# gooofy/zerovox

Hardware: AMD Instinct MI355X
Metric: audio samples/sec + RTF, 128-phoneme zero-shot synth @22.05kHz, 1/2/4/8 GPU (higher is better)
Workload: dtype f16+bf16

## Files before the change

### zerovox_amd/build.py

```python
import os
import subprocess
import sys

HERE = os.path.dirname(os.path.abspath(__file__))
CSRC = os.path.join(HERE, "csrc")
LIB = os.path.join(HERE, "libzvx.so")
KTEST_SRC = os.path.join(os.path.dirname(HERE), "tests", "native", "zvx_ktest.hip")
KTEST_LIB = os.path.join(HERE, "libzvx_ktest.so")
SOURCES = ["gemm.hip", "resstream.hip", "pairstream.hip", "narrowstage.hip", "attention.hip", "ops.hip", "spectral.hip", "zvx.hip"]
UNITS = [("gemm", "gemm.hip", ["-DZVX_GEMM_PART=1"]), ("gemm_resfuse", "gemm.hip", ["-DZVX_GEMM_PART=2"])] + \
        [(s_[:-4], s_, []) for s_ in SOURCES[1:]]
FLAGS = ["--offload-arch=gfx950", "-O3", "-std=c++17", "-fPIC", "-Wall", "-Wno-unused-function", "-Wno-inline-asm"]
EXTRA_FLAGS = {"gemm.hip": ["-fno-honor-nans"], "pairstream.hip": ["-fno-honor-nans"], "narrowstage.hip": ["-fno-honor-nans"], "resstream.hip": ["-fno-honor-nans"] + (["-DRS_PROFILE"] if os.environ.get("ZVX_RS_PROFILE_BUILD") else [])}


def _stale(target, deps):
    if not os.path.exists(target):
        return True
    t = os.path.getmtime(target)
    return any(os.path.getmtime(d) > t for d in deps)


def _parse_resources(text):
    import re
    res, cur = {}, None
    keys = {"TotalSGPRs": "sgprs", "VGPRs": "vgprs", "AGPRs": "agprs", "ScratchSize [bytes/lane]": "scratch", "Occupancy [waves/SIMD]": "occupancy",
            "SGPRs Spill": "sgpr_spill", "VGPRs Spill": "vgpr_spill", "LDS Size [bytes/block]": "lds"}
    for line in text.splitlines():
        m = re.search(r"remark:\s+Function Name: (\S+)", line)
        if m:
            cur = res.setdefault(m.group(1), {})
            continue
        m = re.search(r"remark:\s+([A-Za-z \[\]/]+): (\d+)", line)
        if m and cur is not None and m.group(1).strip() in keys:
            cur[keys[m.group(1).strip()]] = int(m.group(2))
    return res


def resources():
    import json
    out = {}
    for stem, _src, _defs in UNITS:
        f = os.path.join(CSRC, stem + ".resources.json")
        if os.path.exists(f):
            out.update(json.load(open(f)))
    return out


def build(force: bool = False, verbose: bool = True) -> str:
    hipcc = os.environ.get("HIPCC", "/opt/rocm/bin/hipcc")
    headers = [os.path.join(CSRC, "zvx_kernels.h"), os.path.join(CSRC, "mfma_util.h"), os.path.join(CSRC, "stream_plan.h"), os.path.join(os.path.dirname(HERE), "include", "zvx.h")]
    def compile_one(unit):
        stem, src, defs = unit
        s = os.path.join(CSRC, src)
        o = os.path.join(CSRC, stem + ".o")
        rj = os.path.join(CSRC, stem + ".resources.json")
        if force or _stale(o, [s] + headers) or not os.path.exists(rj):
            cmd = [hipcc] + FLAGS + EXTRA_FLAGS.get(src, []) + defs + ["-Rpass-analysis=kernel-resource-usage", "-c", s, "-o", o]
            if verbose:
                print(" ".join(cmd), flush=True)
            p = subprocess.run(cmd, stderr=subprocess.PIPE, text=True)
            lines, keep, skip = p.stderr.splitlines(), [], 0
            for l in lines:
                if "[-Rpass-analysis=kernel-resource-usage]" in l:
                    skip = 2
                elif skip and (l.lstrip().startswith("|") or (l.strip()[:1].isdigit() and " | " in l)):
# ... 43 lines not shown
```

### zerovox_amd/csrc/gemm.hip

```cpp
#include "mfma_util.h"
#include "zvx_kernels.h"

#include <cstring>
#include <type_traits>

#ifndef ZVX_GEMM_PART
#define ZVX_GEMM_PART 0
#endif
#define ZVX_PART_MAIN (ZVX_GEMM_PART != 2)
#define ZVX_PART_RESFUSE (ZVX_GEMM_PART != 1)
#if ZVX_GEMM_PART == 2
extern thread_local bool zvx_gemm_dry_run;
#else
thread_local hipEvent_t zvx_gemm_ev_start = nullptr, zvx_gemm_ev_stop = nullptr;
thread_local bool zvx_gemm_dry_run = false;
#endif
#define g_dry_run zvx_gemm_dry_run

#define ZVX_LAUNCH(...) do { if (!g_dry_run) ZVX_DISPATCH(__VA_ARGS__); } while (0)

namespace zvx {


#define PITCH 80
// ... 1650 lines not shown
        if (a.ntaps == 3) { ZVX_RFP_MODE(3) }
        if (a.ntaps == 7) { ZVX_RFP_MODE(7) }
        if constexpr (C <= 32) { if (a.ntaps == 11) { ZVX_RFP_MODE(11) } }
    }
#undef ZVX_RFP_MODE
#undef ZVX_RFP
    return false;
}

int launch_resfuse(GemmArgs a, hipStream_t stream) {
    if (a.dtype == DT_F32 || !a.Wp || !a.Wp2 || a.N != a.K || a.nheads != 1 || a.wout > 0) return -1;
    if (!(a.ntaps == 3 || a.ntaps == 7 || a.ntaps == 11)) return -1;
    int h1 = 0;
    for (int i = 0; i < a.ntaps; i++) { const int d = a.dv1[i] < 0 ? -a.dv1[i] : a.dv1[i]; if (d > h1) h1 = d; }
    if (h1 > 32) return -1;
    a.halo_l = a.halo_r = h1;
    a.fused = 1;
    if (a.N == 128 && a.no_pairstream != 1) {
        const int h2 = (a.ntaps - 1) / 2, dil = a.dv1[1] - a.dv1[0];
        bool ok = a.alpha == 1.f && a.bias_mode == 1 && !a.post_scale && (!a.out || a.out_dtype == a.dtype) && a.res_mode == 2 && a.res_dtype == a.dtype &&
                  a.res == a.X && a.r_bs == a.x_bs && a.ldr == a.ldx && (!a.accum || a.accum_dtype == a.dtype) && (a.act == ACT_NONE || a.act == ACT_LRELU) &&
                  (a.accum_mode || a.out_scale == 1.f) && a.in_len == a.out_len;
        for (int t = 0; t < a.ntaps; t++) ok = ok && a.dv[t] == t - h2 && a.dv1[t] == (t - h2) * dil;
        if (ok) {
            PairArgs p;
            memset(&p, 0, sizeof p);
            p.X = a.X; p.x_bs = a.x_bs; p.ldx = a.ldx; p.W1 = a.Wp2; p.W2 = a.Wp; p.b1 = a.bias1; p.b2 = a.bias;
            p.C = a.N; p.ntaps = a.ntaps; p.dil = dil;
            p.out = a.out; p.o_bs = a.o_bs; p.ldo = a.ldo;
            p.accum = a.accum; p.a_bs = a.a_bs; p.lda = a.lda; p.accum_mode = a.accum ? a.accum_mode : 0;
            p.slope1 = a.slope1; p.res_inv_slope = a.res_inv_slope; p.out_scale = a.out_scale; p.slope = a.act == ACT_LRELU ? a.slope : 1.f;
            p.f16 = a.dtype == DT_F16;
            p.len = a.out_len; p.M = a.M; p.nbatch = a.nbatch; p.force = a.no_pairstream == 2;
            if (launch_pairstream(p, stream, g_dry_run)) return 23;
        }
    }
    {
        if (a.N == 32 && launch_resfuse_persist_c<32>(a, stream)) return 16;
        if (a.N == 64 && a.ntaps != 11 && launch_resfuse_persist_c<64>(a, stream)) return 17;
        if (a.N == 64 && a.ntaps == 11 && launch_resfuse_persist_c<64, 1>(a, stream)) return 17;
    }
    return -1;
}
#endif
#if ZVX_PART_MAIN

struct Variant { const char* name; int dt, bm, bn; };
static const Variant kVariants[] = {
    {"gemm_bf16_128x128", DT_BF16, 128, 128}, {"gemm_bf16_256x64", DT_BF16, 256, 64},
    {"gemm_bf16_256x32", DT_BF16, 256, 32},   {"gemm_f32_128x128", DT_F32, 128, 128},
    {"gemm_f32_256x64", DT_F32, 256, 64},     {"gemm_f32_256x32", DT_F32, 256, 32},
    {"convslab_bf16_128x256", DT_BF16, 128, 256}, {"convslab_bf16_256x128", DT_BF16, 256, 128},
    {"convslab_bf16_256x64", DT_BF16, 256, 64},   {"convslab_bf16_256x32", DT_BF16, 256, 32},
    {"(unused)", DT_BF16, 0, 0}, {"resfuse_bf16_c8", DT_BF16, 256, 8}, {"resfuse_bf16_c16", DT_BF16, 256, 16}, {"resfuse_bf16_c128", DT_BF16, 64, 128},
    {"convreg_bf16_c32", DT_BF16, 512, 32},       {"convreg_bf16_c64", DT_BF16, 256, 64},
    {"resfuse_bf16_c32", DT_BF16, 256, 32},       {"resfuse_bf16_c64", DT_BF16, 128, 64},
    {"gemm_bf16_64x64", DT_BF16, 64, 64},         {"gemm_f32_64x64", DT_F32, 64, 64},
    {"resstream_bf16_c32", DT_BF16, 64, 32},      {"resstream_bf16_c64", DT_BF16, 32, 64},
    {"convslab_bf16_128x128", DT_BF16, 128, 128},
    {"pairstream_bf16_c128", DT_BF16, 128, 128},
    {"narrowstage_c16", DT_BF16, 256, 16}, {"narrowstage_c8", DT_BF16, 512, 8},
    {"conv2d_persist_c32", DT_BF16, 384, 32}, {"conv2d_persist_c64", DT_BF16, 256, 64},
    {"conv2d_s2_c32", DT_BF16, 256, 64}, {"conv2d_s2_c64", DT_BF16, 128, 128},
    {"rb2fuse_bf16_c32", DT_BF16, 256, 32}, {"rb2fuse_bf16_c64", DT_BF16, 256, 64},
};
const char* gemm_variant_name(int id) { return kVariants[id].name; }
int gemm_num_variants() { return (int)(sizeof(kVariants) / sizeof(kVariants[0])); }


template <int BM, int BN, int WM, int WN, int MINW, int R, int EPI = -1>
static void launch_slab_variant(const GemmArgs& a, dim3 grid, size_t lds, hipStream_t stream) {
    const bool fullk = a.K % SLAB_KC == 0 && a.K2 == 0;
    if constexpr (R == 0 || EPI == -1 || EPI == ZVX_EPI(0, 0, 1) || EPI == ZVX_EPI_FLIP) {
        if (a.dtype == DT_F16) {
            if (fullk) ZVX_LAUNCH((convslab_kernel<BM, BN, WM, WN, true, MINW, R, EPI, 64, true>), grid, dim3(256), lds, stream, a);
            else if constexpr (EPI != ZVX_EPI_FLIP) ZVX_LAUNCH((convslab_kernel<BM, BN, WM, WN, false, MINW, R, EPI, 64, true>), grid, dim3(256), lds, stream, a);
            return;
        }
    }
    if constexpr (EPI < 0 || !(EPI & 16)) {
        if (fullk) ZVX_LAUNCH((convslab_kernel<BM, BN, WM, WN, true, MINW, R, EPI>), grid, dim3(256), lds, stream, a);
        else if constexpr (EPI != ZVX_EPI_FLIP) ZVX_LAUNCH((convslab_kernel<BM, BN, WM, WN, false, MINW, R, EPI>), grid, dim3(256), lds, stream, a);
    }
}

int gemm_epi_mode_of(const GemmArgs& a) {
    if (a.alpha == 1.f && !a.post_scale && a.out && a.out_dtype != a.dtype && a.dtype != DT_F32 && a.out_dtype != DT_F32 && !a.out_split3 && a.bias_mode == 1 && a.bias &&
        (a.act == ACT_NONE || a.act == ACT_LRELU) && !a.res_mode && !(a.accum && a.accum_mode) && a.out_scale == 1.f && a.K % SLAB_KC == 0 && !a.K2) return ZVX_EPI_FLIP;
    if (a.alpha != 1.f || a.post_scale || (a.out && a.out_dtype != a.dtype) || a.dtype == DT_F32 || a.out_split3 || a.bias_mode == 2) return -1;
    const int am = a.accum ? a.accum_mode : 0;
    if (a.dtype == DT_F16 && a.out && !am && a.act == ACT_NONE && a.res_mode <= 1 && (!a.res_mode || a.res_dtype == DT_F16) && (a.res_mode || a.out_scale != 1.f) &&
        (a.bias_mode == 0 || a.bias)) return ZVX_EPI_DEC(a.res_mode ? 1 : 0);
    if (a.bias_mode != 1 || !a.bias) return -1;
    if (a.act != ACT_NONE && a.act != ACT_LRELU) return -1;
    if (a.res_mode && (a.res_mode != 2 || a.res_dtype != a.dtype)) return -1;
    if (am && a.accum_dtype != a.dtype) return -1;
    if (!am && a.out_scale != 1.f) return -1;
    if (!a.out && !(am & 2)) return -1;
    const int e = ZVX_EPI(a.res_mode ? 1 : 0, am, a.out ? 1 : 0);
    switch (e) {
        case ZVX_EPI(0, 0, 1): case ZVX_EPI(1, 0, 1): case ZVX_EPI(1, 2, 0): case ZVX_EPI(1, 3, 0): case ZVX_EPI(1, 1, 1): return e;
    }
    return -1;
}

static int launch_convslab(GemmArgs a, hipStream_t stream) {
    const bool bflat_hint = a.bflat != 0;
// ... 247 lines not shown
```

### zerovox_amd/csrc/zvx.hip

```cpp
#include "../../include/zvx.h"
#include "zvx_kernels.h"
#include "stream_plan.h"

#include <dlfcn.h>
#include <math.h>
#include <cmath>
#include <rccl/rccl.h>
#include <stdarg.h>
#include <stdio.h>
#include <string.h>

#include <algorithm>
#include <map>
#include <sstream>
#include <stdexcept>
#include <string>
#include <vector>

using namespace zvx;

namespace {

struct ZvxError : std::runtime_error {
    int code;
// ... 28 lines not shown
struct zvx_ctx {
    int device = 0;
    hipStream_t stream = nullptr;
    hipStream_t main0 = nullptr;
    hipStream_t comm_stream = nullptr;
    hipStream_t voc_aux[2] = {nullptr, nullptr};
    hipEvent_t voc_ev[3] = {nullptr, nullptr, nullptr};
    int voc_overlap_maxb = 1 << 20;
    int voc_overlap_frames = 28672;
    hipStream_t front_stream = nullptr;
    hipEvent_t ev_front_done = nullptr, ev_mel_free = nullptr, ev_main_join = nullptr;
    int front_overlap = 1;
    bool mel_free_pending = false;
    bool front_dirty_main = true;
    struct HostSlot { void* p = nullptr; size_t cap = 0; hipEvent_t ready = nullptr, done = nullptr; bool pending = false; int B = 0, pcm16 = 0; long stride = 0, need = 0; };
    HostSlot host_slot[2];
    int host_next = 0, host_last = -1;
    hipStream_t copy_stream = nullptr;
    bool copy_is_comm = false;
    hipStream_t aux_stream = nullptr;
    hipEvent_t ev_aux[2] = {nullptr, nullptr};
    int va_overlap_maxb = 1 << 20;
    ncclComm_t comm = nullptr;
    int rank = 0, world = 1;
    hipEvent_t ev_compute = nullptr;
    std::map<const void*, hipEvent_t> gather_fence;
    std::string err;
    std::map<std::string, std::string> cfg;
    std::map<std::string, Tensor> tensors;
    std::vector<float> host_blob;
    std::map<std::string, DevBuf> bufs;
    std::map<const void*, const void*> packed;
    std::map<const void*, const void*> pair_packed;
    int dt = DT_BF16;
    int H = 0, emb_dim = 0, punct_dim = 0, n_phone_rows = 0, n_punct_rows = 0, max_txt_len = 0, max_mel_len = 0;
    int enc_layers = 0, enc_heads = 0, ffn_dim = 0, ffn_k0 = 0, ffn_k1 = 0, vp_dim = 0, vp_k = 0, n_bins = 0;
    int dec_layers = 0, dec_heads = 0, dec_scln = 0, n_mels = 0, hop = 0, res_dim = 0, dec_kind = 0, rn_asp = 1;
    std::vector<int> rn_layers, rn_filters, voc_rates, voc_ksizes, voc_rb_k;
    std::vector<std::vector<int>> voc_rb_d;
    int voc_resblock = 1, voc_c0 = 0;
    int B = 0, Tmax = 0, Lmax = 0;
    std::vector<int> T_host, mel_len_host;
    std::vector<int> in_stage;
    bool have_features = false, have_mel = false;
    int profile = 0;
    int profile_only = -1;
    int rs_prof = 0;
    int enc_split = 0;
    const void* fft_xs_ready = nullptr;
    int norm_fuse_maxb = 1 << 20;
    int dec_sc_fuse = 1;
    int dec_flat = 1;
    int voc_f16_stages = -1;
    int voc_h16_ok = -1;
    int voc_f16 = 1;
    int dec_f16 = 1;
    int use_attn_f32 = 1;
    int use_flash = 1;
    int use_resstream = 1;
    int rs_seg_min = 0;
    int spk_s2_fuse = 1;
    int spk_pool_fuse = 1;
    int slab_small = 2, slab_flat = 1;
    int poison_pads = 0;
    int sat_check = 0;
    unsigned long long* sat_count_dev() { return (unsigned long long*)buf("sat.count", 64); }
    void sat_scan(const void* x, int dt, long bs, int ld, int B, int rows_max, const int* rows, int C) {
        if (sat_check && x && dt == DT_F16) launch_count_sat16(x, bs, ld, B, rows_max, rows, C, sat_count_dev(), stream);
    }
    int use_rb2fuse = 1;
    int use_stagefuse = 1;
    struct NsWeights { void* W = nullptr; float* bias = nullptr; int woff[18] = {0}; };
    std::map<std::string, NsWeights> ns_weights;
    int use_pairstream = 1;
    int shape_log = 0;
    int max_frames = 1 << 18;
    int out_rate = 0;
    struct RsBank { int L = 0, M = 0, half = 0, T = 0, pitch = 0; const float* dev = nullptr; };
    std::map<std::pair<int, int>, RsBank> rs_banks;
    std::map<int, const double*> lim_wins;
    std::map<int, LoudCoef> loud_coefs;
    struct DnTables { int n_fft = 0, log2n = 0, win_length = 0; const float* twid = nullptr; const float* win = nullptr; const double* win2 = nullptr; double den_min = 0; };
    DnTables dn_tab;
    void* join_host = nullptr;
    size_t join_host_cap = 0;
    void* join_pinned(size_t bytes) {
        if (bytes > join_host_cap) {
            if (join_host) { HIPCHK(hipStreamSynchronize(stream)); HIPCHK(hipHostFree(join_host)); join_host = nullptr; join_host_cap = 0; }
            const size_t cap = bytes + bytes / 8 + 256;
            HIPCHK(hipHostMalloc(&join_host, cap, hipHostMallocDefault));
            join_host_cap = cap;
        }
        return join_host;
    }
    hipEvent_t stage_ev[ZVX_T_COUNT][2];
    bool stage_used[ZVX_T_COUNT];
    float stage_ms[ZVX_T_COUNT];
    std::vector<GemmEvent> pending;
    std::vector<zvx_kernel_stat> stats;
    std::string tag = "other";
    std::map<std::string, zvx_kernel_stat> tagstats;
    std::map<std::string, zvx_kernel_stat> namedstats;
    std::vector<hipEvent_t> event_pool;
    std::vector<zvx_stream*> streams;

    int cfg_int(const char* k) const {
// ... 1081 lines not shown
struct VocStage {
    int i, Cin, Cout, rows_in, rows;
    const int* len_in; const int* len;
    int dt_in, dt;
    float next_slope;
};

struct RbConv { std::string name; const Tensor* w = nullptr; const void* packed = nullptr; const float* bias = nullptr; };
struct RbWeights { std::string name; std::vector<RbConv> c1, c2; };
RbWeights voc_rb_weights(zvx_ctx* c, const VocCall& v, const VocStage& s, int j) {
    RbWeights w;
    w.name = "voc.rb" + std::to_string(s.i * v.nk + j);
    auto conv = [&](const char* which, int t) {
        RbConv r;
        r.name = w.name + which + std::to_string(t);
        r.w = &voc_weight(c, r.name + "_w", s.dt);
        auto it = c->packed.find(r.w->dev);
        if (it != c->packed.end()) r.packed = it->second;
        r.bias = c->pf(r.name + "_b");
        return r;
    };
    for (int t = 0; t < (int)c->voc_rb_d[j].size(); t++) {
        if (c->voc_resblock == 1) { w.c1.push_back(conv(".c1_", t)); w.c2.push_back(conv(".c2_", t)); }
        else w.c1.push_back(conv(".c_", t));
    }
    return w;
}

struct StageClose { int accum_mode; bool writes_out; };
StageClose stage_close(int j, int nk) {
    if (nk == 1) return {0, true};
    return {j == 0 ? 2 : (j < nk - 1 ? 3 : 1), j == nk - 1};
}
template <typename Args>
void close_stage(Args& a, const StageClose& cl, const VocCall& v, const VocStage& s) {
    a.accum = cl.accum_mode ? v.XS : nullptr; a.accum_mode = cl.accum_mode; a.a_bs = (long)s.rows * s.Cout; a.lda = s.Cout;
    if (cl.writes_out) { a.out = v.A; a.out_scale = 1.0f / v.nk; a.slope = s.next_slope; }
    else a.out = nullptr;
    if constexpr (std::is_same<Args, GemmArgs>::value) { a.accum_dtype = s.dt; if (cl.writes_out) a.act = ACT_LRELU; }
}

void voc_conv_pre(zvx_ctx* c, const VocCall& v, const void* vin, int dt) {
    const int nm = c->n_mels, Pmax = v.Pmax;
    const int* P_d = v.lens_d + v.B;
    GemmArgs a = gemm_base(dt);
    a.X = vin; a.x_bs = (long)Pmax * nm; a.ldx = nm; a.W = voc_weight(c, "voc.pre_w", dt).dev; a.ldw = nm; a.w_ts = (long)c->voc_c0 * nm;
    a.M = Pmax; a.N = c->voc_c0; a.K = nm; a.nbatch = v.B; a.in_len = P_d; a.out_len = P_d;
    set_taps_1d(a, c->t("voc.pre_w").dim(0), 1);
    a.bias = c->pf("voc.pre_b"); a.bias_mode = 1; a.act = ACT_LRELU; a.slope = 0.1f;
    a.out = v.A; a.o_bs = (long)Pmax * c->voc_c0; a.ldo = c->voc_c0;
    c->gemm(a);
}

void voc_upsample(zvx_ctx* c, const VocCall& v, const VocStage& s) {
    const int u = c->voc_rates[s.i], ku = c->voc_ksizes[s.i], B = v.B, Cin = s.Cin, Cout = s.Cout, rows_in = s.rows_in, dt_in = s.dt_in;
    const std::string up = "voc.up" + std::to_string(s.i);
    GemmArgs a = gemm_base(dt_in);
    a.out_dtype = s.dt;
    a.X = v.A; a.x_bs = (long)rows_in * Cin; a.ldx = Cin; a.ldw = Cin;
    a.M = rows_in; a.K = Cin; a.nbatch = B; a.in_len = s.len_in; a.out_len = s.len_in;
    a.bias_mode = 1; a.act = ACT_LRELU; a.slope = 0.1f;
    a.o_bs = (long)rows_in * u * Cout; a.ldo = u * Cout;
    if (dt_in != DT_F32 && c->has(up + "_wlo")) {
        const int hc = (u / 2) * Cout;
        a.N = hc; a.ntaps = 2; a.w_ts = (long)hc * Cin; a.flops = 2.0 * B * (double)rows_in * Cin * Cout * ku / 2;
        a.W = voc_weight(c, up + "_wlo", dt_in).dev; a.dv[0] = -1; a.dv[1] = 0;
        a.bias = c->pf(up + "_b"); a.out = v.X0;
        c->gemm(a);
        a.Wp = nullptr;
        a.W = voc_weight(c, up + "_whi", dt_in).dev; a.dv[0] = 0; a.dv[1] = 1;
        a.bias = c->pf(up + "_b") + hc; a.out = (char*)v.X0 + (size_t)hc * c->es();
        c->gemm(a);
    } else {
        a.W = voc_weight(c, up + "_w", dt_in).dev; a.w_ts = (long)u * Cout * Cin; a.N = u * Cout;
        a.ntaps = 3; a.dv[0] = -1; a.dv[1] = 0; a.dv[2] = 1;
        a.bias = c->pf(up + "_b"); a.out = v.X0;
        a.flops = 2.0 * B * (double)rows_in * Cin * Cout * ku;
        c->gemm(a);
    }
}

const zvx_ctx::NsWeights& voc_narrow_weights(zvx_ctx* c, const VocCall& v, const VocStage& s) {
    const int Cout = s.Cout, nk = v.nk;
    const std::string key = "voc.ns." + std::to_string(s.i) + (s.dt == DT_F16 ? ".h16" : "");
    auto it = c->ns_weights.find(key);
    if (it != c->ns_weights.end()) return it->second;
    zvx_ctx::NsWeights nw;
    int nfrag = 0;
    for (int j = 0; j < nk; j++) for (int q = 0; q < 6; q++) { nw.woff[6 * j + q] = nfrag; nfrag += narrowstage_steps(Cout, c->voc_rb_k[j]); }
    nw.W = c->buf(key + ".w", (size_t)nfrag * 1024);
    nw.bias = c->fbuf(key + ".b", (size_t)6 * nk * Cout);
    for (int j = 0; j < nk; j++) {
        const RbWeights w = voc_rb_weights(c, v, s, j);
        for (int t = 0; t < 3; t++)
            for (int q = 0; q < 2; q++) {
                const RbConv& cv = q ? w.c2[t] : w.c1[t];
                if (cv.w->dims.size() != 3 || cv.w->dim(0) != c->voc_rb_k[j] || cv.w->dim(1) != Cout || cv.w->dim(2) != Cout) fail(ZVX_E_MANIFEST, "weights: '%s' has an unexpected shape", cv.name.c_str());
                const int ci = 6 * j + 2 * t + q;
                launch_pack_narrow(cv.w->dev, c->voc_rb_k[j], Cout, (char*)nw.W + (size_t)nw.woff[ci] * 1024, c->stream);
                HIPCHK(hipMemcpyAsync(nw.bias + (size_t)ci * Cout, cv.bias, (size_t)Cout * 4, hipMemcpyDeviceToDevice, c->stream));
            }
    }
    return c->ns_weights.emplace(key, nw).first->second;
}

bool voc_narrow_stage(zvx_ctx* c, const VocCall& v, const VocStage& s) {
    const int Cout = s.Cout, nk = v.nk, rows = s.rows;
    if (!c->use_stagefuse || c->sat_check || c->voc_resblock != 1 || s.dt == DT_F32 || (Cout != 16 && Cout != 8) || nk < 1 || nk > 3) return false;
    for (int j = 0; j < nk; j++) if (c->voc_rb_d[j].size() != 3) return false;
// ... 1807 lines not shown
void zvx_destroy(zvx_ctx* c) {
    if (!c) return;
    (void)hipSetDevice(c->device);
    if (c->front_stream) (void)hipStreamSynchronize(c->front_stream);
    if (c->stream) (void)hipStreamSynchronize(c->stream);
    while (!c->streams.empty()) stream_free(c->streams.back());
    zvx_comm_destroy(c);
    for (int i = 0; i < 2; i++) { if (c->arena[i].p) (void)hipHostFree(c->arena[i].p); if (c->arena[i].ev) (void)hipEventDestroy(c->arena[i].ev); }
    if (c->copy_stream && !c->copy_is_comm) { (void)hipStreamSynchronize(c->copy_stream); (void)hipStreamDestroy(c->copy_stream); }
    for (auto& hs : c->host_slot) { if (hs.p) (void)hipHostFree(hs.p); if (hs.ready) (void)hipEventDestroy(hs.ready); if (hs.done) (void)hipEventDestroy(hs.done); }
    if (c->join_host) (void)hipHostFree(c->join_host);
    for (int i = 0; i < 2; i++) if (c->voc_aux[i]) { (void)hipStreamSynchronize(c->voc_aux[i]); (void)hipStreamDestroy(c->voc_aux[i]); }
    for (int i = 0; i < 3; i++) if (c->voc_ev[i]) (void)hipEventDestroy(c->voc_ev[i]);
    if (c->aux_stream) { (void)hipStreamSynchronize(c->aux_stream); (void)hipStreamDestroy(c->aux_stream); (void)hipEventDestroy(c->ev_aux[0]); (void)hipEventDestroy(c->ev_aux[1]); }
    if (c->front_stream) {
        (void)hipStreamSynchronize(c->front_stream); (void)hipStreamDestroy(c->front_stream);
        (void)hipEventDestroy(c->ev_front_done); (void)hipEventDestroy(c->ev_mel_free); (void)hipEventDestroy(c->ev_main_join);
    }
    for (auto& kv : c->bufs) if (kv.second.base) (void)hipFree(kv.second.base);
    for (auto e : c->event_pool) (void)hipEventDestroy(e);
    if (c->stream) {
        for (int s = 0; s < ZVX_T_COUNT; s++) { (void)hipEventDestroy(c->stage_ev[s][0]); (void)hipEventDestroy(c->stage_ev[s][1]); }
        (void)hipStreamDestroy(c->stream);
    }
    delete c;
}

const char* zvx_last_error(const zvx_ctx* c) { return c ? c->err.c_str() : g_create_error.c_str(); }

namespace {

struct Switch { const char* key; int zvx_ctx::*v; bool (*ok)(int64_t); };
bool flag(int64_t v) { return v == 0 || v == 1; }
bool count(int64_t v) { return v >= 0 && v <= INT32_MAX; }
const Switch kSwitches[] = {
    {"profile", &zvx_ctx::profile, [](int64_t v) { return v >= 0 && v <= 2; }},
    {"profile_only", &zvx_ctx::profile_only, [](int64_t v) { return v >= -1 && v < gemm_num_variants(); }},
    {"shape_log", &zvx_ctx::shape_log, flag},
    {"rs_prof", &zvx_ctx::rs_prof, flag},
    {"f16_sat_check", &zvx_ctx::sat_check, flag},
    {"poison_pads", &zvx_ctx::poison_pads, flag},
    {"max_frames", &zvx_ctx::max_frames, [](int64_t v) { return v >= 1 && v <= (1 << 24); }},
    {"enc_split", &zvx_ctx::enc_split, [](int64_t v) { return v >= 0 && v <= 2; }},
    {"attn_f32", &zvx_ctx::use_attn_f32, flag},
    {"flash", &zvx_ctx::use_flash, flag},
    {"front_overlap", &zvx_ctx::front_overlap, [](int64_t v) { return v >= 0 && v <= 2; }},
    {"va_overlap_maxb", &zvx_ctx::va_overlap_maxb, count},
    {"dec_f16", &zvx_ctx::dec_f16, flag},
    {"dec_flat", &zvx_ctx::dec_flat, flag},
    {"dec_sc_fuse", &zvx_ctx::dec_sc_fuse, flag},
    {"norm_fuse_maxb", &zvx_ctx::norm_fuse_maxb, count},
    {"voc_f16", &zvx_ctx::voc_f16, flag},
    {"voc_f16_stages", &zvx_ctx::voc_f16_stages, [](int64_t v) { return v >= -1 && v <= INT32_MAX; }},
    {"voc_overlap_maxb", &zvx_ctx::voc_overlap_maxb, count},
    {"voc_overlap_frames", &zvx_ctx::voc_overlap_frames, count},
    {"stagefuse", &zvx_ctx::use_stagefuse, flag},
    {"rb2fuse", &zvx_ctx::use_rb2fuse, flag},
    {"resstream", &zvx_ctx::use_resstream, flag},
    {"rs_seg_min", &zvx_ctx::rs_seg_min, [](int64_t v) { return v >= -1 && v <= INT32_MAX; }},
    {"pairstream", &zvx_ctx::use_pairstream, [](int64_t v) { return v == -1 || v == 0 || v == 1 || v == 3; }},
    {"slab_small", &zvx_ctx::slab_small, [](int64_t v) { return (v & ~32) >= 0 && (v & ~32) <= 2; }},
    {"slab_flat", &zvx_ctx::slab_flat, flag},
    {"spk_pool_fuse", &zvx_ctx::spk_pool_fuse, flag},
    {"spk_s2_fuse", &zvx_ctx::spk_s2_fuse, flag},
    {"out_rate", &zvx_ctx::out_rate, count},
};
const Switch* find_switch(const char* key) {
    for (const Switch& s : kSwitches) if (!strcmp(s.key, key)) return &s;
    return nullptr;
}

}

int64_t zvx_get_int(const zvx_ctx* c, const char* key) {
    if (!c || !key) return -1;
    if (const Switch* s = find_switch(key)) return c->*s->v;
    const std::string k(key);
    if (k == "precision") return c->dt == DT_F32 ? 1 : 0;
    if (k == "hidden") return c->H;
    if (k == "n_mels") return c->n_mels;
    if (k == "hop") return c->hop;
    if (k == "device") return c->device;
    if (k == "dec_kind") return c->dec_kind;
    if (k == "Lmax") return c->Lmax;
    if (k == "f16_sat_events") {
        zvx_ctx* m = const_cast<zvx_ctx*>(c);
        unsigned long long n = 0;
        if (hipSetDevice(m->device) != hipSuccess) return -1;
        try { unsigned long long* d = m->sat_count_dev(); m->sync(); if (hipMemcpy(&n, d, sizeof n, hipMemcpyDeviceToHost) != hipSuccess) return -1; } catch (...) { return -1; }
        return (int64_t)n;
    }
    if (k == "host_slot") return c->host_last;
    if (k.rfind("variant_id:", 0) == 0) { for (int i = 0; i < gemm_num_variants(); i++) if (k.substr(11) == gemm_variant_name(i)) return i; return -1; }
    auto it = c->cfg.find(k);
    if (it != c->cfg.end()) return atoll(it->second.c_str());
    return -1;
}

zvx_status zvx_set_int(zvx_ctx* c, const char* key, int64_t value) {
    return guarded(c, [&] {
        if (!key) fail(ZVX_E_INVALID, "key is NULL");
        const Switch* s = find_switch(key);
        if (!s) fail(ZVX_E_INVALID, "unknown option '%s'", key);
        if (!s->ok(value)) fail(ZVX_E_INVALID, "option '%s' does not take the value %lld", key, (long long)value);
        const std::string k(key);
        if (k == "out_rate" && value) {
// ... 550 lines not shown
```

### zerovox_amd/csrc/zvx_kernels.h

```cpp
#pragma once
#include <hip/hip_runtime.h>
#include <hip/hip_ext.h>
#include <stdint.h>
#include <atomic>
#include <mutex>
#include <set>
#include <utility>

extern thread_local hipEvent_t zvx_gemm_ev_start, zvx_gemm_ev_stop;
#define ZVX_DISPATCH(kernel, grid, block, lds, stream, ...) \
    do { if (zvx_gemm_ev_start) hipExtLaunchKernelGGL(kernel, grid, block, lds, stream, zvx_gemm_ev_start, zvx_gemm_ev_stop, 0, __VA_ARGS__); \
         else hipLaunchKernelGGL(kernel, grid, block, lds, stream, __VA_ARGS__); } while (0)

namespace zvx {

inline void profile_events(hipEvent_t start, hipEvent_t stop) { zvx_gemm_ev_start = start; zvx_gemm_ev_stop = stop; }

typedef unsigned short bf16_t;

enum DType { DT_F32 = 0, DT_BF16 = 1, DT_F16 = 2 };
static inline size_t dtype_size(int dt) { return dt == DT_F32 ? 4 : 2; }
inline int num_cus() {
    static const int n = [] { int dev = 0, v = 0; if (hipGetDevice(&dev) != hipSuccess || hipDeviceGetAttribute(&v, hipDeviceAttributeMultiprocessorCount, dev) != hipSuccess || v <= 0) v = 256; return v; }();
    return n;
// ... 64 lines not shown
const char* gemm_variant_name(int id);
int gemm_num_variants();

struct StreamArgs {
    const void* X; long x_bs; int ldx;
    const void* W1[3]; const void* W2[3];
    const float* b1[3]; const float* b2[3];
    int dil[3];
    int C, ntaps, npair;
    void* out; long o_bs; int ldo;
    void* accum; long a_bs; int lda; int accum_mode;
    float slope1, res_inv_slope, out_scale, slope;
    const int* len; int M, nbatch;
    int S, nseg;
    int dX0, dT, dX[3];
    double flops;
    long long* prof;
    int seg_min;
    int f16;
};
int launch_resstream(StreamArgs a, hipStream_t stream, bool dry_run);

struct PairArgs {
    const void* X; long x_bs; int ldx;
    const void* W1; const void* W2;
    const float* b1; const float* b2;
    int C, ntaps, dil;
    void* out; long o_bs; int ldo;
    void* accum; long a_bs; int lda; int accum_mode;
    float slope1, res_inv_slope, out_scale, slope;
    const int* len; int M, nbatch;
    int force;
    int f16;
    int S, nseg, DX, DT, G0;
    long long* prof;
};
bool launch_pairstream(PairArgs a, hipStream_t stream, bool dry_run);

struct StageArgs {
    const void* X; long x_bs; int ldx;
    const void* W;
    int woff[18];
    const float* bias;
    int C, nk, ks[3], dil[3][3];
    void* out; long o_bs; int ldo;
    float slope1, res_inv_slope, slope;
    const int* len; int M, nbatch;
    int f16;
};
bool launch_narrowstage(const StageArgs& a, hipStream_t stream, bool dry_run);
int narrowstage_steps(int C, int k);
void launch_pack_narrow(const void* w16 , int k, int C, void* out, hipStream_t s);

struct FlashArgs {
    const void* qk; long qk_bs; int ldq; int k_off;
    const void* vt; long vt_bs; int ldv;
    void* out; long o_bs; int ldo;
    const int* len; int L, D, nheads, nbatch;
    float scale;
    int f16;
    long long* prof;
};
bool launch_flash_attention(const FlashArgs& a, hipStream_t stream, bool dry_run);
struct AttnF32Args {
    const float* qkv; long bs; int ld; int q_off, k_off, v_off;
    float* out; long o_bs; int ldo;
    unsigned short* planes; int planes_C;
    int planes_f16;
    const int* len; int L, D, nheads, nbatch;
    float scale;
};
bool launch_attention_f32(const AttnF32Args& a, hipStream_t stream, bool dry_run);

void launch_instnorm_fused(const void* x, int x_dt, int ldx, void* y, int y_dt, int ldy, int B, int Lmax, const int* L, int C, float eps,
                           float* mean, float* rstd, const float* gamma, const float* beta, long g_bs, int one_plus, int act, float slope, hipStream_t s);
void launch_transpose16(const void* in, int ld_in, void* out, int ld_out, int B, int rows, int C, hipStream_t s, const int* len = nullptr);
void launch_f32_to_bf16(const float* in, bf16_t* out, size_t n, hipStream_t s);
void launch_zero_tail_cols(void* x, int es, long ld, long bs, int B, int rows, int cols, const int* len, hipStream_t s);
void launch_cast(const void* in, int in_dt, void* out, int out_dt, size_t n, hipStream_t s);

void launch_split3(const float* x, int ldx, void* out, int B, int rows_max, const int* rows, int C, hipStream_t s, int f16 = 0);
void launch_split3_weights(const float* w, void* out, long nrows, int K, hipStream_t s, int f16 = 0, float scale = 1.f);
void launch_absmax(const float* x, size_t n, float* out , hipStream_t s);

void launch_embed(const int* phoneme, const int* puncts, const float* emb, int emb_dim, const float* pemb,
                  int pemb_dim, const float* pe, float* out, int B, int Tmax, const int* T, hipStream_t s);

void launch_layernorm(const void* x, int x_dt, int ldx, void* y, int y_dt, int ldy, int B, int rows_max,
                      const int* rows, int C, int mode, float eps, const float* gamma, const float* beta,
                      const float* bg, long bg_bs, const float* post_add, hipStream_t s, void* split_planes = nullptr, int planes_f16 = 0);

void launch_softmax_rows(const float* scores, int lds, void* P, int p_dt, int ldp, int nbatch, int nheads,
                         int Lmax, const int* len, hipStream_t s);

void launch_rowdot(const float* x, int ldx, const float* w, float bias, float* out, int B, int Tmax,
                   const int* T, int C, hipStream_t s);

void launch_bucket_embed_add(const float* pred, const float* table, int nbins, float* x, int ldx, int C,
                             int* idx_out, int B, int Tmax, const int* T, hipStream_t s);

void launch_durations(const int* forced, const float* logd, int* dur, int* cum, int* mel_len, int B, int Tmax,
                      const int* T, hipStream_t s);

void launch_bucket_embed_add_ctl(const float* pred, const float* shift, const float* range, const float* target, const float* table,
                                 int nbins, float* x, int ldx, int C, int* idx_out, int B, int Tmax, const int* T, hipStream_t s);
void launch_durations_q16(const int* forced, const float* logd, const int* q, int* dur, int* cum, int* mel_len, int B, int Tmax,
// ... 159 lines not shown
```

Before: 348.2 million.

## Add dedicated transposed-conv upsample kernel for small vocoder stages

Adds a new MFMA kernel for the vocoder's transposed-convolution upsample (kernel = 2×rate). It stages input rows in LDS and streams prepacked weights through a register ring, then fuses bias, leaky ReLU and output packing with a permlane swap for coalesced stores. It is enabled by default for stages with Cin ≤ 256 and replaces the generic GEMM path there. It relies on a packed weight layout found via c->packed, and falls back to the GEMM path if the shape is unsupported.

```diff
diff --git a/zerovox_amd/build.py b/zerovox_amd/build.py
--- a/zerovox_amd/build.py
+++ b/zerovox_amd/build.py
@@ -7,11 +7,11 @@
 LIB = os.path.join(HERE, "libzvx.so")
 KTEST_SRC = os.path.join(os.path.dirname(HERE), "tests", "native", "zvx_ktest.hip")
 KTEST_LIB = os.path.join(HERE, "libzvx_ktest.so")
-SOURCES = ["gemm.hip", "resstream.hip", "pairstream.hip", "narrowstage.hip", "attention.hip", "ops.hip", "spectral.hip", "zvx.hip"]
+SOURCES = ["gemm.hip", "resstream.hip", "pairstream.hip", "narrowstage.hip", "convt.hip", "attention.hip", "ops.hip", "spectral.hip", "zvx.hip"]
 UNITS = [("gemm", "gemm.hip", ["-DZVX_GEMM_PART=1"]), ("gemm_resfuse", "gemm.hip", ["-DZVX_GEMM_PART=2"])] + \
         [(s_[:-4], s_, []) for s_ in SOURCES[1:]]
 FLAGS = ["--offload-arch=gfx950", "-O3", "-std=c++17", "-fPIC", "-Wall", "-Wno-unused-function", "-Wno-inline-asm"]
-EXTRA_FLAGS = {"gemm.hip": ["-fno-honor-nans"], "pairstream.hip": ["-fno-honor-nans"], "narrowstage.hip": ["-fno-honor-nans"], "resstream.hip": ["-fno-honor-nans"] + (["-DRS_PROFILE"] if os.environ.get("ZVX_RS_PROFILE_BUILD") else [])}
+EXTRA_FLAGS = {"gemm.hip": ["-fno-honor-nans"], "pairstream.hip": ["-fno-honor-nans"], "narrowstage.hip": ["-fno-honor-nans"], "convt.hip": ["-fno-honor-nans"], "resstream.hip": ["-fno-honor-nans"] + (["-DRS_PROFILE"] if os.environ.get("ZVX_RS_PROFILE_BUILD") else [])}
 
 
 def _stale(target, deps):
diff --git a/zerovox_amd/csrc/convt.hip b/zerovox_amd/csrc/convt.hip
--- /dev/null
+++ b/zerovox_amd/csrc/convt.hip
@@ -0,0 +1,146 @@
+#include "mfma_util.h"
+#include "zvx_kernels.h"
+
+namespace zvx {
+
+#define CONVT_VARIANT 10
+
+template <int CIN, int COUT, int U, int BM, int TN, bool HIN, bool HOUT>
+__global__ __launch_bounds__(256, 2) void convt_kernel(const ConvtArgs a) {
+    constexpr int PITCH = CIN * 2 + 16;
+    constexpr int SR = BM + 2, CPR = CIN / 8;
+    constexpr int NIT = (SR * CPR + 255) / 256;
+    constexpr int NG = U * COUT / 32 / TN;
+    constexpr int WN = NG < 4 ? NG : 4, WM = 4 / WN;
+    constexpr int RPW = BM / WM, TM = RPW / 32, GPW = NG / WN;
+    constexpr int NKC = CIN / 64, STEPS = NKC * 8;
+    static_assert(CIN % 64 == 0 && (COUT / 32) % TN == 0 && U % 2 == 0 && BM % (32 * WM) == 0 && NG % WN == 0 && 4 % WN == 0, "shape");
+    extern __shared__ __attribute__((aligned(16))) unsigned char slab[];
+
+    const int tid = threadIdx.x, lane = tid & 63, wave = __builtin_amdgcn_readfirstlane(tid >> 6);
+    const int wc = wave % WN, wr = wave / WN;
+    const int b = blockIdx.y, m0 = blockIdx.x * BM;
+    int len = a.len ? a.len[b] : a.M;
+    if (len > a.M) len = a.M;
+    if (m0 >= len) return;
+
+    auto group_base = [&](int gi) {
+        const int tile = ((gi < GPW ? gi : 0) * WN + wc) * TN;
+        const int hi = (tile * 32 / COUT) >= U / 2;
+        return (const unsigned char*)a.Wp + ((long)tile * NKC * 12 + hi * 4) * 1024 + lane * 16;
+    };
+    auto wload = [&](uint4 (&dst)[TN], const unsigned char* base, int s) {
+#pragma unroll
+        for (int i = 0; i < TN; i++) dst[i] = *(const uint4*)(base + ((i * NKC * 12 + (s >> 3) * 12 + ((s >> 2) & 1) * 4 + (s & 3)) * 1024));
+    };
+    const unsigned char* wt = group_base(0);
+    uint4 ring[4][TN];
+#pragma unroll
+    for (int s = 0; s < 4; s++) wload(ring[s], wt, s);
+
+    {
+        const unsigned short* Xp = (const unsigned short*)a.X + (long)b * a.x_bs;
+        uint4 sv[NIT];
+#pragma unroll
+        for (int i = 0; i < NIT; i++) {
+            const int c = tid + i * 256;
+            const int row = c / CPR, q = c % CPR;
+            const int g = m0 - 1 + row;
+            sv[i] = make_uint4(0, 0, 0, 0);
+            if (c < SR * CPR && g >= 0 && g < len) sv[i] = *(const uint4*)(Xp + (long)g * CIN + q * 8);
+        }
+#pragma unroll
+        for (int i = 0; i < NIT; i++) {
+            const int c = tid + i * 256;
+            if (c < SR * CPR) *(uint4*)(slab + (c / CPR) * PITCH + (c % CPR) * 16) = sv[i];
+        }
+    }
+    __syncthreads();
+
+    const float slope = a.slope;
+    const int h4 = 4 * (lane >> 5);
+    unsigned short* const obase = (unsigned short*)a.out + (long)b * a.o_bs;
+    for (int gi = 0; gi < GPW; gi++) {
+        const int tile0 = (gi * WN + wc) * TN;
+        const int hi = (tile0 * 32 / COUT) >= U / 2;
+        const unsigned char* const wnext = group_base(gi + 1);
+        const unsigned char* const xrow = slab + (wr * RPW + (lane & 31) + hi) * PITCH + (lane >> 5) * 16;
+        f32x16 acc[TN][TM];
+#pragma unroll
+        for (int i = 0; i < TN; i++)
+#pragma unroll
+            for (int j = 0; j < TM; j++)
+#pragma unroll
+                for (int e = 0; e < 16; e++) acc[i][j][e] = 0.f;
+#pragma unroll
+        for (int s = 0; s < STEPS; s++) {
+            uint4 wf[TN];
+#pragma unroll
+            for (int i = 0; i < TN; i++) wf[i] = ring[s & 3][i];
+            if (s + 4 < STEPS) wload(ring[s & 3], wt, s + 4); else wload(ring[s & 3], wnext, s + 4 - STEPS);
+            const int xo = ((s >> 2) & 1) * PITCH + (s >> 3) * 128 + (s & 3) * 32;
+#pragma unroll
+            for (int j = 0; j < TM; j++) {
+                const uint4 xf = *(const uint4*)(xrow + j * 32 * PITCH + xo);
+#pragma unroll
+                for (int i = 0; i < TN; i++) acc[i][j] = mfma16<HIN>(wf[i], xf, acc[i][j]);
+            }
+        }
+        wt = wnext;
+
+#pragma unroll
+        for (int i = 0; i < TN; i++) {
+            const int n0 = (tile0 + i) * 32;
+            float4 bb[4];
+#pragma unroll
+            for (int g = 0; g < 4; g++) bb[g] = *(const float4*)(a.bias + n0 + 8 * g + h4);
+#pragma unroll
+            for (int j = 0; j < TM; j++) {
+                const int r = m0 + wr * RPW + j * 32 + (lane & 31);
+                const bool ok = r < len;
+                uint2 pk[4];
+#pragma unroll
+                for (int g = 0; g < 4; g++) {
+                    const f32x2 v01 = lrelu2((f32x2){acc[i][j][4 * g], acc[i][j][4 * g + 1]} + (f32x2){bb[g].x, bb[g].y}, slope);
+                    const f32x2 v23 = lrelu2((f32x2){acc[i][j][4 * g + 2], acc[i][j][4 * g + 3]} + (f32x2){bb[g].z, bb[g].w}, slope);
+                    pk[g].x = HOUT ? pack_f16x2_sat(v01.x, v01.y) : pack_bf16x2(v01.x, v01.y);
+                    pk[g].y = HOUT ? pack_f16x2_sat(v23.x, v23.y) : pack_bf16x2(v23.x, v23.y);
+                }
+                unsigned short* const op = obase + (long)(ok ? r : m0) * (U * COUT) + n0;
+                typedef __attribute__((ext_vector_type(2))) unsigned u32x2_t;
+#pragma unroll
+                for (int pr = 0; pr < 2; pr++) {
+                    const u32x2_t sx = __builtin_amdgcn_permlane32_swap(pk[2 * pr].x, pk[2 * pr + 1].x, false, false);
+                    const u32x2_t sy = __builtin_amdgcn_permlane32_swap(pk[2 * pr].y, pk[2 * pr + 1].y, false, false);
+                    if (ok) *(u32x4*)(op + 8 * (2 * pr + (lane >> 5))) = (u32x4){sx.x, sy.x, sx.y, sy.y};
+                }
+            }
+        }
+    }
+}
+
+template <int CIN, int COUT, int U, int BM, int TN>
+static int launch_convt_shape(const ConvtArgs& a, hipStream_t stream, bool dry_run) {
+    constexpr size_t lds = (size_t)(BM + 2) * (CIN * 2 + 16);
+    static_assert(2 * lds <= 160 * 1024, "two workgroups per CU");
+    if (dry_run) return CONVT_VARIANT;
+    const dim3 grid((a.M + BM - 1) / BM, a.nbatch), block(256);
+#define CONVT_GO(HI_, HO_) do { auto kfn = convt_kernel<CIN, COUT, U, BM, TN, HI_, HO_>; \
+        if (lds > 64 * 1024 && !lds_opt_in((const void*)kfn)) return -1; \
+        ZVX_DISPATCH(kfn, grid, block, lds, stream, a); } while (0)
+    if (a.f16_in) { if (a.f16_out) CONVT_GO(true, true); else CONVT_GO(true, false); }
+    else { if (a.f16_out) CONVT_GO(false, true); else CONVT_GO(false, false); }
+#undef CONVT_GO
+    return CONVT_VARIANT;
+}
+
+int launch_convt(const ConvtArgs& a, hipStream_t stream, bool dry_run) {
+    if (!a.X || !a.Wp || !a.bias || !a.out || a.k != 2 * a.u || a.M <= 0 || a.nbatch <= 0 || a.nbatch > 65535) return -1;
+    if (a.Cin == 512 && a.Cout == 256 && a.u == 8) return launch_convt_shape<512, 256, 8, 64, 1>(a, stream, dry_run);
+    if (a.Cin == 256 && a.Cout == 128 && a.u == 8) return launch_convt_shape<256, 128, 8, 128, 2>(a, stream, dry_run);
+    if (a.Cin == 128 && a.Cout == 64 && a.u == 2) return launch_convt_shape<128, 64, 2, 256, 1>(a, stream, dry_run);
+    if (a.Cin == 64 && a.Cout == 32 && a.u == 2) return launch_convt_shape<64, 32, 2, 256, 1>(a, stream, dry_run);
+    return -1;
+}
+
+}
diff --git a/zerovox_amd/csrc/gemm.hip b/zerovox_amd/csrc/gemm.hip
--- a/zerovox_amd/csrc/gemm.hip
+++ b/zerovox_amd/csrc/gemm.hip
@@ -1726,7 +1726,7 @@
     {"gemm_f32_256x64", DT_F32, 256, 64},     {"gemm_f32_256x32", DT_F32, 256, 32},
     {"convslab_bf16_128x256", DT_BF16, 128, 256}, {"convslab_bf16_256x128", DT_BF16, 256, 128},
     {"convslab_bf16_256x64", DT_BF16, 256, 64},   {"convslab_bf16_256x32", DT_BF16, 256, 32},
-    {"(unused)", DT_BF16, 0, 0}, {"resfuse_bf16_c8", DT_BF16, 256, 8}, {"resfuse_bf16_c16", DT_BF16, 256, 16}, {"resfuse_bf16_c128", DT_BF16, 64, 128},
+    {"convt_rows", DT_BF16, 0, 0} , {"resfuse_bf16_c8", DT_BF16, 256, 8}, {"resfuse_bf16_c16", DT_BF16, 256, 16}, {"resfuse_bf16_c128", DT_BF16, 64, 128},
     {"convreg_bf16_c32", DT_BF16, 512, 32},       {"convreg_bf16_c64", DT_BF16, 256, 64},
     {"resfuse_bf16_c32", DT_BF16, 256, 32},       {"resfuse_bf16_c64", DT_BF16, 128, 64},
     {"gemm_bf16_64x64", DT_BF16, 64, 64},         {"gemm_f32_64x64", DT_F32, 64, 64},
diff --git a/zerovox_amd/csrc/zvx.hip b/zerovox_amd/csrc/zvx.hip
--- a/zerovox_amd/csrc/zvx.hip
+++ b/zerovox_amd/csrc/zvx.hip
@@ -104,6 +104,7 @@
     int dec_sc_fuse = 1;
     int dec_flat = 1;
     int voc_f16_stages = -1;
+    int voc_convt = 1;
     int voc_h16_ok = -1;
     int voc_f16 = 1;
     int dec_f16 = 1;
@@ -1291,9 +1292,32 @@
     c->gemm(a);
 }
 
+bool convt_stage_pays(int Cin, int u) { (void)u; return Cin <= 256; }
+
 void voc_upsample(zvx_ctx* c, const VocCall& v, const VocStage& s) {
     const int u = c->voc_rates[s.i], ku = c->voc_ksizes[s.i], B = v.B, Cin = s.Cin, Cout = s.Cout, rows_in = s.rows_in, dt_in = s.dt_in;
     const std::string up = "voc.up" + std::to_string(s.i);
+    if (c->voc_convt && dt_in != DT_F32 && s.dt != DT_F32 && !c->sat_check && (c->voc_convt == 2 || convt_stage_pays(Cin, u))) {
+        const Tensor& w = voc_weight(c, up + "_w", dt_in);
+        auto it = c->packed.find(w.dev);
+        ConvtArgs t{};
+        t.X = v.A; t.x_bs = (long)rows_in * Cin; t.Wp = it != c->packed.end() ? it->second : nullptr; t.bias = c->pf(up + "_b");
+        t.out = v.X0; t.o_bs = (long)rows_in * u * Cout; t.len = s.len_in; t.M = rows_in; t.nbatch = B;
+        t.Cin = Cin; t.Cout = Cout; t.u = u; t.k = ku; t.f16_in = dt_in == DT_F16; t.f16_out = s.dt == DT_F16; t.slope = 0.1f;
+        const int id = launch_convt(t, c->stream, true);
+        if (id >= 0) {
+            c->profiled([&] { return id; }, [&] {
+                const int id2 = launch_convt(t, c->stream, false);
+                if (id2 < 0) fail(ZVX_E_INVALID, "launch_convt rejected a shape its dry run accepted (Cin=%d Cout=%d u=%d)", Cin, Cout, u);
+                return id2;
+            }, [&](GemmEvent& ev) {
+                const double rows = (double)rows_in * B, esz = 2.0;
+                ev.flops = 2.0 * rows * Cin * Cout * ku; ev.rows = (long)rows; ev.N = u * Cout; ev.K = Cin; ev.taps = 2; ev.res = 0; ev.fused = 0;
+                ev.bytes = rows * Cin * esz + (double)u * Cout * Cin * 2 * esz + rows * u * Cout * esz;
+            });
+            return;
+        }
+    }
     GemmArgs a = gemm_base(dt_in);
     a.out_dtype = s.dt;
     a.X = v.A; a.x_bs = (long)rows_in * Cin; a.ldx = Cin; a.ldw = Cin;
@@ -3207,6 +3231,7 @@
     {"norm_fuse_maxb", &zvx_ctx::norm_fuse_maxb, count},
     {"voc_f16", &zvx_ctx::voc_f16, flag},
     {"voc_f16_stages", &zvx_ctx::voc_f16_stages, [](int64_t v) { return v >= -1 && v <= INT32_MAX; }},
+    {"voc_convt", &zvx_ctx::voc_convt, [](int64_t v) { return v >= 0 && v <= 2; }},
     {"voc_overlap_maxb", &zvx_ctx::voc_overlap_maxb, count},
     {"voc_overlap_frames", &zvx_ctx::voc_overlap_frames, count},
     {"stagefuse", &zvx_ctx::use_stagefuse, flag},
diff --git a/zerovox_amd/csrc/zvx_kernels.h b/zerovox_amd/csrc/zvx_kernels.h
--- a/zerovox_amd/csrc/zvx_kernels.h
+++ b/zerovox_amd/csrc/zvx_kernels.h
@@ -140,6 +140,18 @@
 int narrowstage_steps(int C, int k);
 void launch_pack_narrow(const void* w16 , int k, int C, void* out, hipStream_t s);
 
+struct ConvtArgs {
+    const void* X; long x_bs;
+    const void* Wp;
+    const float* bias;
+    void* out; long o_bs;
+    const int* len; int M, nbatch;
+    int Cin, Cout, u, k;
+    int f16_in, f16_out;
+    float slope;
+};
+int launch_convt(const ConvtArgs& a, hipStream_t stream, bool dry_run);
+
 struct FlashArgs {
     const void* qk; long qk_bs; int ldq; int k_off;
     const void* vt; long vt_bs; int ldv;
```

Measured after the change: 350.7 million (median of 6 runs). About the same (+0.7%).
